# mahyarnajibi/SNIPER

Measured on AMD Instinct MI355X. Metric: train chips/sec (512x512, R101), higher is better.
Workload: dtype f16; 1 GPU; ResNet-101 Faster-RCNN SNIPER 3-scale, batch 20 x 512x512 fp16 per GPU (BASELINE configs[1]); step = GPU anchor labelling + fwd + bwd + grad all-reduce + SGD on HBM-resident chips (epoch chip generation / box assignment and image decode+resize are outside the step); f16 MFMA operands, f32 accumulation / losses / master weights; chips_per_gpu=20, global_batch=20, parallelism=dp1

## Files before the change

### sniper_amd/csrc/nn_ops.hip

```cpp
#include "common.h"
#include "softmax_grad.h"
#include <algorithm>

__global__ __launch_bounds__(256) void pack_stem_kernel(const float *__restrict__ x, half_t *__restrict__ out, int N, int C,
                                                        int H, int W, int Hp, int Wp, int pad_t, int pad_l,
                                                        const float *__restrict__ scale, const float *__restrict__ shift) {
  const long total = (long)N * Hp * Wp;
  for (long i = (long)blockIdx.x * blockDim.x + threadIdx.x; i < total; i += (long)gridDim.x * blockDim.x) {
    const int xp = (int)(i % Wp);
    const long t = i / Wp;
    const int yp = (int)(t % Hp), n = (int)(t / Hp);
    const int sy = yp - pad_t, sx = xp - pad_l;
    half_t v[4] = {0, 0, 0, 0};
    if ((unsigned)sy < (unsigned)H && (unsigned)sx < (unsigned)W) {
      for (int c = 0; c < C && c < 4; ++c) {
        float f = x[(((long)n * C + c) * H + sy) * W + sx];
        if (scale) f = f * scale[c] + shift[c];
        v[c] = (half_t)f;
      }
    }
    *reinterpret_cast<uint2 *>(out + i * 4) = *reinterpret_cast<uint2 *>(v);
  }
}

// ... 1121 lines not shown

__global__ __launch_bounds__(256) void softmax_rows_bwd_kernel(const float *__restrict__ p, const float *__restrict__ label,
                                                               float *__restrict__ g, long outer, int K, int R, SnDiv dK, float ignore,
                                                               int use_ignore, float grad_scale, int normalize_valid,
                                                               const int *__restrict__ valid_count) {
  softmax_bwd_rows(p, label, g, outer, K, R, dK, ignore, use_ignore, softmax_grad_mul(grad_scale, normalize_valid, valid_count));
}

SN_EXPORT int sn_softmax_fwd(const float *x, float *p, long outer, int K, long inner, sn_stream_t stream) {
  SN_REQUIRE(x && p && outer > 0 && K > 0 && inner > 0, "sn_softmax_fwd: bad arguments");
  if (softmax_rows_ok(x, p, K, inner)) {
    const int R = softmax_rows_per_block(K);
    SN_REQUIRE((outer + R - 1) / R < (1l << 31), "sn_softmax_fwd: too many rows");
    hipLaunchKernelGGL(softmax_rows_fwd_kernel, dim3((unsigned)((outer + R - 1) / R)), dim3(256), (size_t)R * (K | 1) * sizeof(float),
                       sn_stream(stream), x, p, outer, K, R, sn_div_make((unsigned)K));
  } else {
    hipLaunchKernelGGL(softmax_fwd_kernel, dim3(ew_blocks(outer * inner)), dim3(256), 0, sn_stream(stream), x, p, outer, K, inner);
  }
  SN_CHECK_LAUNCH();
  return SN_OK;
}

int sn_softmax_count_valid(const float *label, long n, float ignore_label, int use_ignore, int *ws, hipStream_t s) {
  SN_HIP(hipMemsetAsync(ws, 0, sizeof(int), s));
  hipLaunchKernelGGL(count_valid_kernel, dim3(sn_blocks(n, 256)), dim3(256), 0, s, label, n, use_ignore ? ignore_label : -1e30f, ws);
  SN_CHECK_LAUNCH();
  return SN_OK;
}

SN_EXPORT int sn_softmax_output_bwd(const float *p, const float *label, float *grad, long outer, int K, long inner,
                                    float ignore_label, int use_ignore, float grad_scale, int normalize_valid, int *ws,
                                    sn_stream_t stream) {
  SN_REQUIRE(p && label && grad && ws, "sn_softmax_output_bwd: null pointer");
  hipStream_t s = sn_stream(stream);
  if (normalize_valid) {
    const int rc = sn_softmax_count_valid(label, outer * inner, ignore_label, use_ignore, ws, s);
    if (rc != SN_OK) return rc;
  }
  if (softmax_rows_ok(p, grad, K, inner)) {
    const int R = softmax_rows_per_block(K);
    SN_REQUIRE((outer + R - 1) / R < (1l << 31), "sn_softmax_output_bwd: too many rows");
    hipLaunchKernelGGL(softmax_rows_bwd_kernel, dim3((unsigned)((outer + R - 1) / R)), dim3(256), 0, s, p, label, grad, outer, K, R,
                       sn_div_make((unsigned)K), ignore_label, use_ignore, grad_scale, normalize_valid, ws);
  } else {
    hipLaunchKernelGGL(softmax_bwd_kernel, dim3(ew_blocks(outer * inner)), dim3(256), 0, s, p, label, grad, outer, K, inner,
                       ignore_label, use_ignore, grad_scale, normalize_valid, ws);
  }
  SN_CHECK_LAUNCH();
  return SN_OK;
}

__global__ __launch_bounds__(256) void smooth_l1_kernel(const float *__restrict__ pred, const float *__restrict__ target,
                                                        const float *__restrict__ weight, float *__restrict__ loss,
                                                        float *__restrict__ dpred, long n, float sigma, float grad_scale) {
  const float s2 = sigma * sigma, th = 1.f / s2;
  for (long i = (long)blockIdx.x * blockDim.x + threadIdx.x; i < n; i += (long)gridDim.x * blockDim.x) {
    const float d = pred[i] - target[i], w = weight[i];
    const float ad = fabsf(d);
    if (loss) loss[i] = w * (ad < th ? 0.5f * s2 * d * d : ad - 0.5f * th);
    if (dpred) dpred[i] = grad_scale * w * (ad < th ? s2 * d : (d > 0.f ? 1.f : (d < 0.f ? -1.f : 0.f)));
  }
}

SN_EXPORT int sn_smooth_l1_loss(const float *pred, const float *target, const float *weight, float *loss, float *dpred,
                                long n, float sigma, float grad_scale, sn_stream_t stream) {
  SN_REQUIRE(pred && target && weight && n > 0, "sn_smooth_l1_loss: bad arguments");
  hipLaunchKernelGGL(smooth_l1_kernel, dim3(ew_blocks(n)), dim3(256), 0, sn_stream(stream), pred, target, weight, loss, dpred,
                     n, sigma, grad_scale);
  SN_CHECK_LAUNCH();
  return SN_OK;
}

__global__ __launch_bounds__(256) void sgd_kernel(float *__restrict__ w32, const float *__restrict__ grad, float *__restrict__ mom,
                                                  half_t *__restrict__ w16, long n, float lr, float wd, float momentum,
                                                  float rescale) {
  for (long i = (long)blockIdx.x * blockDim.x + threadIdx.x; i < n; i += (long)gridDim.x * blockDim.x) {
    const float w = w32[i];
    const float g = rescale * grad[i] + wd * w;
    const float m = momentum * mom[i] - lr * g;
    mom[i] = m;
    const float nw = w + m;
    w32[i] = nw;
    if (w16) w16[i] = (half_t)nw;
  }
}

SN_EXPORT int sn_sgd_mom_update(float *w32, const float *grad, float *mom, void *w16, long n, float lr, float wd,
                                float momentum, float rescale, sn_stream_t stream) {
  SN_REQUIRE(w32 && grad && mom && n >= 0, "sn_sgd_mom_update: bad arguments");
  if (n == 0) return SN_OK;
  hipLaunchKernelGGL(sgd_kernel, dim3(ew_blocks(n)), dim3(256), 0, sn_stream(stream), w32, grad, mom, (half_t *)w16, n, lr, wd,
                     momentum, rescale);
  SN_CHECK_LAUNCH();
  return SN_OK;
}

__device__ __forceinline__ float sgd_statement(float w, float gr, float m_old, float lr, float wd, float momentum, float rescale,
                                               float &nm) {
  const float g = rescale * gr + wd * w;
  nm = momentum * m_old - lr * g;
  return w + nm;
}

__device__ __forceinline__ float sgd_statement_guarded(float w, float gr, float m_old, float lr, float wd, float momentum, float rescale,
                                                       float coef, float clip, float &nm) {
  float u = rescale * (coef * gr);
  if (clip > 0.f) u = fminf(fmaxf(u, -clip), clip);
  const float g = u + wd * w;
  nm = momentum * m_old - lr * g;
  return w + nm;
}

__global__ __launch_bounds__(256) void sgd_dev_kernel(float *__restrict__ w32, const float *__restrict__ grad,
                                                      float *__restrict__ mom, half_t *__restrict__ w16, long n,
                                                      const float *__restrict__ hyper, float lr_mult, float wd_mult) {
  const float lr = hyper[0] * lr_mult, wd = hyper[1] * wd_mult, momentum = hyper[2], rescale = hyper[3];
  for (long i = (long)blockIdx.x * blockDim.x + threadIdx.x; i < n; i += (long)gridDim.x * blockDim.x) {
    float m;
    const float nw = sgd_statement(w32[i], grad[i], mom[i], lr, wd, momentum, rescale, m);
    mom[i] = m;
    w32[i] = nw;
    if (w16) w16[i] = (half_t)nw;
  }
}

__global__ __launch_bounds__(256) void sgd_dev_vec4_kernel(float4 *__restrict__ w32, const float4 *__restrict__ grad,
                                                           float4 *__restrict__ mom, half_t *__restrict__ w16, long n4,
                                                           const float *__restrict__ hyper, float lr_mult, float wd_mult) {
  const float lr = hyper[0] * lr_mult, wd = hyper[1] * wd_mult, momentum = hyper[2], rescale = hyper[3];
  for (long i = (long)blockIdx.x * blockDim.x + threadIdx.x; i < n4; i += (long)gridDim.x * blockDim.x) {
    const float4 w = w32[i], g4 = grad[i], m4 = mom[i];
    float4 nm, nw;
    nw.x = sgd_statement(w.x, g4.x, m4.x, lr, wd, momentum, rescale, nm.x);
    nw.y = sgd_statement(w.y, g4.y, m4.y, lr, wd, momentum, rescale, nm.y);
    nw.z = sgd_statement(w.z, g4.z, m4.z, lr, wd, momentum, rescale, nm.z);
    nw.w = sgd_statement(w.w, g4.w, m4.w, lr, wd, momentum, rescale, nm.w);
    mom[i] = nm;
    w32[i] = nw;
    if (w16) {
      half4 h;
      h[0] = (half_t)nw.x; h[1] = (half_t)nw.y; h[2] = (half_t)nw.z; h[3] = (half_t)nw.w;
      *reinterpret_cast<half4 *>(w16 + 4 * i) = h;
    }
  }
}

SN_EXPORT int sn_sgd_mom_update_dev(float *w32, const float *grad, float *mom, void *w16, long n, const float *d_hyper,
                                    float lr_mult, float wd_mult, sn_stream_t stream) {
  SN_REQUIRE(w32 && grad && mom && d_hyper && n >= 0, "sn_sgd_mom_update_dev: bad arguments");
  if (n == 0) return SN_OK;
  auto scalar = [&](long from, long count) {
    hipLaunchKernelGGL(sgd_dev_kernel, dim3(ew_blocks(count)), dim3(256), 0, sn_stream(stream), w32 + from, grad + from,
                       mom + from, w16 ? (half_t *)w16 + from : (half_t *)nullptr, count, d_hyper, lr_mult, wd_mult);
  };
  long head = (long)(((16 - ((uintptr_t)w32 & 15)) & 15) / 4);
  if (head > n) head = n;
  const bool same = (((uintptr_t)(w32 + head) | (uintptr_t)(grad + head) | (uintptr_t)(mom + head)) & 15) == 0 &&
                    (w16 == nullptr || ((uintptr_t)((half_t *)w16 + head) & 7) == 0);
  if (!same) {
    scalar(0, n);
    SN_CHECK_LAUNCH();
    return SN_OK;
  }
  if (head > 0) scalar(0, head);
  const long n4 = (n - head) / 4;
  if (n4 > 0)
    hipLaunchKernelGGL(sgd_dev_vec4_kernel, dim3(ew_blocks(n4)), dim3(256), 0, sn_stream(stream), (float4 *)(w32 + head),
                       (const float4 *)(grad + head), (float4 *)(mom + head), w16 ? (half_t *)w16 + head : (half_t *)nullptr, n4,
                       d_hyper, lr_mult, wd_mult);
  const long done = head + 4 * n4;
  if (done < n) scalar(done, n - done);
  SN_CHECK_LAUNCH();
  return SN_OK;
}

__global__ __launch_bounds__(256) void sgd_guard_kernel(float *__restrict__ w32, const float *__restrict__ grad,
                                                        float *__restrict__ mom, half_t *__restrict__ w16, long n,
                                                        const float *__restrict__ hyper, float lr_mult, float wd_mult, float clip,
                                                        const double *__restrict__ state) {
  if (state[2] != 0.0) return;
  const float coef = (float)state[1];
  const float lr = hyper[0] * lr_mult, wd = hyper[1] * wd_mult, momentum = hyper[2], rescale = hyper[3];
  if (coef == 1.f && !(clip > 0.f)) {
    for (long i = (long)blockIdx.x * blockDim.x + threadIdx.x; i < n; i += (long)gridDim.x * blockDim.x) {
      float m;
      const float nw = sgd_statement(w32[i], grad[i], mom[i], lr, wd, momentum, rescale, m);
      mom[i] = m;
      w32[i] = nw;
      if (w16) w16[i] = (half_t)nw;
    }
    return;
  }
  for (long i = (long)blockIdx.x * blockDim.x + threadIdx.x; i < n; i += (long)gridDim.x * blockDim.x) {
    float m;
    const float nw = sgd_statement_guarded(w32[i], grad[i], mom[i], lr, wd, momentum, rescale, coef, clip, m);
    mom[i] = m;
    w32[i] = nw;
    if (w16) w16[i] = (half_t)nw;
  }
}

__global__ __launch_bounds__(256) void sgd_guard_vec4_kernel(float4 *__restrict__ w32, const float4 *__restrict__ grad,
                                                             float4 *__restrict__ mom, half_t *__restrict__ w16, long n4,
                                                             const float *__restrict__ hyper, float lr_mult, float wd_mult,
                                                             float clip, const double *__restrict__ state) {
  if (state[2] != 0.0) return;
  const float coef = (float)state[1];
  const float lr = hyper[0] * lr_mult, wd = hyper[1] * wd_mult, momentum = hyper[2], rescale = hyper[3];
  if (coef == 1.f && !(clip > 0.f)) {
    for (long i = (long)blockIdx.x * blockDim.x + threadIdx.x; i < n4; i += (long)gridDim.x * blockDim.x) {
      const float4 w = w32[i], g4 = grad[i], m4 = mom[i];
      float4 nm, nw;
      nw.x = sgd_statement(w.x, g4.x, m4.x, lr, wd, momentum, rescale, nm.x);
      nw.y = sgd_statement(w.y, g4.y, m4.y, lr, wd, momentum, rescale, nm.y);
      nw.z = sgd_statement(w.z, g4.z, m4.z, lr, wd, momentum, rescale, nm.z);
      nw.w = sgd_statement(w.w, g4.w, m4.w, lr, wd, momentum, rescale, nm.w);
      mom[i] = nm;
      w32[i] = nw;
      if (w16) {
        half4 h;
        h[0] = (half_t)nw.x; h[1] = (half_t)nw.y; h[2] = (half_t)nw.z; h[3] = (half_t)nw.w;
        *reinterpret_cast<half4 *>(w16 + 4 * i) = h;
      }
    }
    return;
  }
  for (long i = (long)blockIdx.x * blockDim.x + threadIdx.x; i < n4; i += (long)gridDim.x * blockDim.x) {
    const float4 w = w32[i], g4 = grad[i], m4 = mom[i];
    float4 nm, nw;
    nw.x = sgd_statement_guarded(w.x, g4.x, m4.x, lr, wd, momentum, rescale, coef, clip, nm.x);
    nw.y = sgd_statement_guarded(w.y, g4.y, m4.y, lr, wd, momentum, rescale, coef, clip, nm.y);
    nw.z = sgd_statement_guarded(w.z, g4.z, m4.z, lr, wd, momentum, rescale, coef, clip, nm.z);
    nw.w = sgd_statement_guarded(w.w, g4.w, m4.w, lr, wd, momentum, rescale, coef, clip, nm.w);
    mom[i] = nm;
    w32[i] = nw;
    if (w16) {
      half4 h;
      h[0] = (half_t)nw.x; h[1] = (half_t)nw.y; h[2] = (half_t)nw.z; h[3] = (half_t)nw.w;
      *reinterpret_cast<half4 *>(w16 + 4 * i) = h;
    }
  }
}

SN_EXPORT int sn_sgd_mom_update_guarded_dev(float *w32, const float *grad, float *mom, void *w16, long n, const float *d_hyper,
                                            float lr_mult, float wd_mult, float clip_gradient, const double *d_state,
                                            sn_stream_t stream) {
  SN_REQUIRE(w32 && grad && mom && d_hyper && d_state && n >= 0, "sn_sgd_mom_update_guarded_dev: bad arguments");
  SN_REQUIRE(clip_gradient == clip_gradient, "sn_sgd_mom_update_guarded_dev: clip_gradient is NaN");
  SN_REQUIRE(((uintptr_t)d_state & 7) == 0, "sn_sgd_mom_update_guarded_dev: d_state must be 8-byte aligned");
  if (n == 0) return SN_OK;
  auto scalar = [&](long from, long count) {
    hipLaunchKernelGGL(sgd_guard_kernel, dim3(ew_blocks(count)), dim3(256), 0, sn_stream(stream), w32 + from, grad + from,
                       mom + from, w16 ? (half_t *)w16 + from : (half_t *)nullptr, count, d_hyper, lr_mult, wd_mult, clip_gradient,
                       d_state);
  };
  long head = (long)(((16 - ((uintptr_t)w32 & 15)) & 15) / 4);
  if (head > n) head = n;
  const bool same = (((uintptr_t)(w32 + head) | (uintptr_t)(grad + head) | (uintptr_t)(mom + head)) & 15) == 0 &&
                    (w16 == nullptr || ((uintptr_t)((half_t *)w16 + head) & 7) == 0);
  if (!same) {
    scalar(0, n);
    SN_CHECK_LAUNCH();
    return SN_OK;
  }
  if (head > 0) scalar(0, head);
  const long n4 = (n - head) / 4;
  if (n4 > 0)
    hipLaunchKernelGGL(sgd_guard_vec4_kernel, dim3(ew_blocks(n4)), dim3(256), 0, sn_stream(stream), (float4 *)(w32 + head),
                       (const float4 *)(grad + head), (float4 *)(mom + head), w16 ? (half_t *)w16 + head : (half_t *)nullptr, n4,
                       d_hyper, lr_mult, wd_mult, clip_gradient, d_state);
  const long done = head + 4 * n4;
  if (done < n) scalar(done, n - done);
  SN_CHECK_LAUNCH();
  return SN_OK;
}

__global__ __launch_bounds__(256) void weight_oti_to_ito_kernel(const float *__restrict__ w, half_t *__restrict__ wt, int O, int T,
                                                                int I, int Opad) {
  const long total = (long)Opad * T * I;
  for (long i = (long)blockIdx.x * blockDim.x + threadIdx.x; i < total; i += (long)gridDim.x * blockDim.x) {
    const int o = (int)(i % Opad);
    const long r = i / Opad;
    const int t = (int)(r % T), ci = (int)(r / T);
    wt[i] = o < O ? (half_t)w[((long)o * T + t) * I + ci] : (half_t)0;
  }
}

SN_EXPORT int sn_weight_transpose(const float *w_oti, void *wt_ito_f16, int O, int T, int I, int O_pad, sn_stream_t stream) {
  SN_REQUIRE(w_oti && wt_ito_f16 && O > 0 && T > 0 && I > 0 && O_pad >= O, "sn_weight_transpose: bad arguments");
  hipLaunchKernelGGL(weight_oti_to_ito_kernel, dim3(ew_blocks((long)O_pad * T * I)), dim3(256), 0, sn_stream(stream), w_oti,
                     (half_t *)wt_ito_f16, O, T, I, O_pad);
  SN_CHECK_LAUNCH();
  return SN_OK;
}

struct WtDesc {
  const float *src;
  half_t *dst;
  int O, T, I, Opad, tile0, tiles_o, tiles_i, pad_;
};
static_assert(sizeof(WtDesc) == 48, "WtDesc layout is part of the C ABI (sn_weight_transpose_batched)");

__global__ __launch_bounds__(256) void weight_transpose_batched_kernel(const WtDesc *__restrict__ desc, int nd) {
  __shared__ float sm[64][65];
  const int tile = blockIdx.x;
  int lo = 0, hi = nd - 1;
  while (lo < hi) {
    const int mid = (lo + hi + 1) >> 1;
    if (desc[mid].tile0 <= tile) lo = mid; else hi = mid - 1;
  }
  const WtDesc d = desc[lo];
  const int local = tile - d.tile0, per_t = d.tiles_o * d.tiles_i;
  const int t = local / per_t, rem = local - t * per_t;
  const int o0 = (rem / d.tiles_i) * 64, i0 = (rem % d.tiles_i) * 64;
  const int c = threadIdx.x & 63, r = threadIdx.x >> 6;
#pragma unroll
  for (int k = 0; k < 16; ++k) {
    const int o = o0 + r + 4 * k, ci = i0 + c;
    sm[r + 4 * k][c] = (o < d.O && ci < d.I) ? d.src[((size_t)o * d.T + t) * d.I + ci] : 0.f;
  }
  __syncthreads();
#pragma unroll
  for (int k = 0; k < 16; ++k) {
    const int ci = i0 + r + 4 * k, o = o0 + c;
    if (ci < d.I && o < d.Opad) d.dst[((size_t)ci * d.T + t) * d.Opad + o] = (half_t)sm[c][r + 4 * k];
  }
}

SN_EXPORT int sn_weight_transpose_batched(const void *desc, int n_desc, int total_tiles, sn_stream_t stream) {
  SN_REQUIRE(desc && n_desc > 0 && total_tiles > 0, "sn_weight_transpose_batched: bad arguments");
  hipLaunchKernelGGL(weight_transpose_batched_kernel, dim3(total_tiles), dim3(256), 0, sn_stream(stream), (const WtDesc *)desc,
                     n_desc);
  SN_CHECK_LAUNCH();
  return SN_OK;
}

__global__ __launch_bounds__(256) void ew_f32_kernel(const float *__restrict__ a, const float *__restrict__ b, float *__restrict__ out,
                                                     long n, int op, float scalar) {
  for (long i = (long)blockIdx.x * blockDim.x + threadIdx.x; i < n; i += (long)gridDim.x * blockDim.x) {
    float v;
    switch (op) {
      case 0: v = a[i] - b[i]; break;
      case 1: v = a[i] + b[i]; break;
      case 2: v = a[i] * b[i]; break;
      case 3: v = a[i] * scalar; break;
      default: v = scalar; break;
    }
    out[i] = v;
  }
}

SN_EXPORT int sn_ew_f32(const float *a, const float *b, float *out, long n, int op, float scalar, sn_stream_t stream) {
  SN_REQUIRE(out && n > 0 && op >= 0 && op <= 4, "sn_ew_f32: bad arguments");
  SN_REQUIRE(op == 4 || a, "sn_ew_f32: null a");
  SN_REQUIRE(op > 2 || b, "sn_ew_f32: null b");
  hipLaunchKernelGGL(ew_f32_kernel, dim3(ew_blocks(n)), dim3(256), 0, sn_stream(stream), a, b, out, n, op, scalar);
  SN_CHECK_LAUNCH();
  return SN_OK;
}

template <typename T>
__global__ __launch_bounds__(256) void bias_grad_kernel(const T *__restrict__ dy, float *__restrict__ db, float *__restrict__ part,
                                                        long rows, int C, int ld, long rows_per_block) {
  const long r0 = (long)blockIdx.y * rows_per_block, r1 = min(rows, r0 + rows_per_block);
  const int c = blockIdx.x * 64 + (threadIdx.x & 63);
  const int rl = threadIdx.x >> 6;
  float s = 0.f;
  if (c < C)
    for (long r = r0 + rl; r < r1; r += 4) s += (float)dy[r * ld + c];
  __shared__ float red[4][64];
  red[rl][threadIdx.x & 63] = s;
  __syncthreads();
  if (rl == 0 && c < C) {
    const float t = (red[0][threadIdx.x] + red[1][threadIdx.x]) + (red[2][threadIdx.x] + red[3][threadIdx.x]);
    if (part) part[(size_t)blockIdx.y * C + c] = t;
    else db[c] += t;
  }
}

__global__ __launch_bounds__(256) void bias_grad_vec8_kernel(const half_t *__restrict__ dy, float *__restrict__ db, float *__restrict__ part,
                                                             long rows, int C, int ld, long rows_per_block) {
  const long r0 = (long)blockIdx.y * rows_per_block, r1 = min(rows, r0 + rows_per_block);
  const int lane = threadIdx.x & 63, rl = threadIdx.x >> 6;
  const int c = (blockIdx.x * 64 + lane) * 8;
  float s[8] = {0.f, 0.f, 0.f, 0.f, 0.f, 0.f, 0.f, 0.f};
  if (c < C) {
    long r = r0 + rl;
    for (; r + 12 < r1; r += 16) {
      half8 v[4];
#pragma unroll
      for (int u = 0; u < 4; ++u) v[u] = *reinterpret_cast<const half8 *>(dy + (r + 4 * u) * ld + c);
#pragma unroll
      for (int u = 0; u < 4; ++u)
#pragma unroll
        for (int j = 0; j < 8; ++j) s[j] += (float)v[u][j];
    }
    for (; r < r1; r += 4) {
      const half8 v = *reinterpret_cast<const half8 *>(dy + r * ld + c);
#pragma unroll
      for (int j = 0; j < 8; ++j) s[j] += (float)v[j];
    }
  }
  __shared__ float red[4][64][9];
#pragma unroll
  for (int j = 0; j < 8; ++j) red[rl][lane][j] = s[j];
  __syncthreads();
  if (rl == 0 && c < C) {
#pragma unroll
    for (int j = 0; j < 8; ++j) {
      if (c + j >= C) break;
      const float t = (red[0][lane][j] + red[1][lane][j]) + (red[2][lane][j] + red[3][lane][j]);
      if (part) part[(size_t)blockIdx.y * C + c + j] = t;
      else db[c + j] += t;
    }
  }
}

static int bias_grad_blocks(long rows, long *rows_per_block) {
  int by = (int)((rows + 255) / 256);
  if (by > 96) by = 96;
  if (by < 1) by = 1;
  *rows_per_block = (rows + by - 1) / by;
  return (int)((rows + *rows_per_block - 1) / *rows_per_block);
}

SN_EXPORT size_t sn_bias_grad_workspace_bytes(long rows, int C) {
  if (rows <= 0 || C <= 0) return 0;
  long rpb;
  int by = bias_grad_blocks(rows, &rpb);
  if (by > 1) by = (int)std::max<long>(by, std::min<long>(128, (rows + 63) / 64));
  return by > 1 ? sn_align(sizeof(float) * (size_t)by * C) : 0;
}

SN_EXPORT int sn_bias_grad(const void *dy, float *db, long rows, int C, int ld, int dtype, void *ws, size_t ws_bytes,
                           sn_stream_t stream) {
  SN_REQUIRE(dy && db && rows > 0 && C > 0, "sn_bias_grad: bad arguments");
  long rpb;
  int by = bias_grad_blocks(rows, &rpb);
  const bool vec8 = dtype == 0 && ld % 8 == 0 && sn_div_up(C, 8) * 8 <= ld && ((uintptr_t)dy % 16) == 0;
  if (vec8 && by > 1 && sn_div_up(C, 512) * by < 256) {
    by = (int)std::min<long>(std::min<long>(128, (rows + 63) / 64), by * 4L);
    if (ws && ws_bytes < sizeof(float) * (size_t)by * C) by = bias_grad_blocks(rows, &rpb);
    rpb = (rows + by - 1) / by;
  }
  float *part = nullptr;
  if (by > 1) {
    if (ws && ws_bytes >= sizeof(float) * (size_t)by * C) part = (float *)ws;
    else { by = 1; rpb = rows; }
  }
  dim3 grid(sn_div_up(C, 64), by);
  hipStream_t s = sn_stream(stream);
  if (vec8)
    hipLaunchKernelGGL(bias_grad_vec8_kernel, dim3(sn_div_up(C, 512), by), dim3(256), 0, s, (const half_t *)dy, db, part, rows, C, ld, rpb);
  else if (dtype == 0)
    hipLaunchKernelGGL((bias_grad_kernel<half_t>), grid, dim3(256), 0, s, (const half_t *)dy, db, part, rows, C, ld, rpb);
  else
    hipLaunchKernelGGL((bias_grad_kernel<float>), grid, dim3(256), 0, s, (const float *)dy, db, part, rows, C, ld, rpb);
  SN_CHECK_LAUNCH();
  return part ? sn_partial_sum(part, by, C, db, s) : SN_OK;
}
```

### sniper_amd/csrc/proposal.hip

```cpp
#include "common.h"

extern "C" int sn_nms_batch(const float *, const int32_t *, int, int, int, float, int, void *, int32_t *, int32_t *, sn_stream_t);
extern "C" size_t sn_nms_workspace_bytes(int, int);

struct PropLayout {
  int total, sort_n, pre, post;
  size_t boxes_all, keys, sorted, nvalid, keep, nkeep, nms, bytes;
};

static int next_pow2(int v) { int p = 1; while (p < v) p <<= 1; return p; }

static PropLayout prop_layout(int B, int A, int Fh, int Fw, int pre, int post) {
  PropLayout L;
  L.total = A * Fh * Fw;
  L.sort_n = next_pow2(L.total);
  L.pre = pre < L.total ? pre : L.total;
  L.post = post < L.pre ? post : L.pre;
  size_t off = 0;
  L.boxes_all = off; off += sn_align((size_t)B * L.total * 4 * sizeof(float));
  L.keys = off; off += sn_align((size_t)B * L.sort_n * sizeof(unsigned long long));
  L.sorted = off; off += sn_align((size_t)B * L.pre * 5 * sizeof(float));
  L.nvalid = off; off += sn_align((size_t)B * sizeof(int32_t));
  L.keep = off; off += sn_align((size_t)B * L.post * sizeof(int32_t));
  L.nkeep = off; off += sn_align((size_t)B * sizeof(int32_t));
  L.nms = off; off += sn_nms_workspace_bytes(B, L.pre);
  L.bytes = off;
  return L;
}

SN_EXPORT size_t sn_proposal_workspace_bytes(int B, int A, int Fh, int Fw, int pre_nms_top_n, int post_nms_top_n) {
  return prop_layout(B, A, Fh, Fw, pre_nms_top_n, post_nms_top_n).bytes;
}

__global__ __launch_bounds__(256) void proposal_decode_kernel(const float *__restrict__ cls_prob, const float *__restrict__ bbox_pred,
                                                              const float *__restrict__ im_info, const float *__restrict__ base,
                                                              int A, int Fh, int Fw, int stride, float min_size, int total, int sort_n,
                                                              float *__restrict__ boxes_all, unsigned long long *__restrict__ keys) {
  const int b = blockIdx.y;
  const int i = blockIdx.x * blockDim.x + threadIdx.x;
  if (i >= sort_n) return;
  unsigned long long *kb = keys + (size_t)b * sort_n;
  if (i >= total) { kb[i] = ~0ull; return; }
  const int cell = i / A, a = i - cell * A;
  const int h = cell / Fw, w = cell - h * Fw;
  const int FF = Fh * Fw;
  const float score0 = cls_prob[((size_t)b * 2 + 1) * A * FF + (size_t)a * FF + cell];
  const float *bp = bbox_pred + ((size_t)b * 4 * A + 4 * a) * FF + cell;
  const float dx = bp[0], dy = bp[FF], dw = bp[2 * FF], dh = bp[3 * FF];
  const float ax1 = base[4 * a] + (float)(w * stride), ay1 = base[4 * a + 1] + (float)(h * stride);
  const float ax2 = base[4 * a + 2] + (float)(w * stride), ay2 = base[4 * a + 3] + (float)(h * stride);
  const float aw = ax2 - ax1 + 1.0f, ah = ay2 - ay1 + 1.0f;
  const float cx = ax1 + 0.5f * (aw - 1.0f), cy = ay1 + 0.5f * (ah - 1.0f);
  const float pcx = dx * aw + cx, pcy = dy * ah + cy;
  const float pw = (float)exp((double)dw) * aw, ph = (float)exp((double)dh) * ah;
  float x1 = pcx - 0.5f * (pw - 1.0f), y1 = pcy - 0.5f * (ph - 1.0f);
  float x2 = pcx + 0.5f * (pw - 1.0f), y2 = pcy + 0.5f * (ph - 1.0f);
  const float im_h = im_info[3 * b], im_w = im_info[3 * b + 1], im_s = im_info[3 * b + 2];
  x1 = fmaxf(fminf(x1, im_w - 1.0f), 0.f); y1 = fmaxf(fminf(y1, im_h - 1.0f), 0.f);
  x2 = fmaxf(fminf(x2, im_w - 1.0f), 0.f); y2 = fmaxf(fminf(y2, im_h - 1.0f), 0.f);
  float score = score0;
  const float ms = min_size * im_s;
  if ((x2 - x1 + 1.0f) < ms || (y2 - y1 + 1.0f) < ms) score = -1.0f;
  float *o = boxes_all + ((size_t)b * total + i) * 4;
  o[0] = x1; o[1] = y1; o[2] = x2; o[3] = y2;
  kb[i] = ((unsigned long long)(~sn_float_key(score)) << 32) | (unsigned)i;
}

__global__ __launch_bounds__(1024) void bitonic_sort_kernel(unsigned long long *__restrict__ keys, int n) {
  unsigned long long *k = keys + (size_t)blockIdx.x * n;
  for (int size = 2; size <= n; size <<= 1) {
    for (int j = size >> 1; j > 0; j >>= 1) {
      for (int t = threadIdx.x; t < (n >> 1); t += blockDim.x) {
        const int lo = 2 * t - (t & (j - 1));
        const int hi = lo + j;
        const bool up = (lo & size) == 0;
        const unsigned long long a = k[lo], c = k[hi];
        if ((a > c) == up) { k[lo] = c; k[hi] = a; }
      }
      __syncthreads();
    }
  }
}

constexpr int kSelThreads = 1024, kSelRegKeys = 32;
template <bool REG>
__global__ __launch_bounds__(kSelThreads) void topk_select_sort_kernel(unsigned long long *__restrict__ keys, int n, int K, int P2) {
  extern __shared__ __attribute__((aligned(16))) unsigned long long sel_buf[];
  __shared__ unsigned hist[256];
  __shared__ unsigned long long s_prefix, s_mask;
  __shared__ int s_need, s_cnt, s_done;
  unsigned long long *k = keys + (size_t)blockIdx.x * n;
  const int tid = threadIdx.x;
  unsigned long long kreg[REG ? kSelRegKeys : 1];
  if constexpr (REG) {
#pragma unroll
    for (int u = 0; u < kSelRegKeys; ++u) {
      const int i = u * kSelThreads + tid;
      kreg[u] = i < n ? k[i] : 0ull;
    }
  }
  const int iters = REG ? (n + kSelThreads - 1) / kSelThreads : 0;
  if (tid == 0) { s_prefix = 0ull; s_mask = 0ull; s_need = K; s_cnt = 0; s_done = 0; }
  __syncthreads();
  for (int shift = 56; shift >= 0; shift -= 8) {
    if (tid < 256) hist[tid] = 0u;
    __syncthreads();
    if (s_done) break;
    const unsigned long long prefix = s_prefix, mask = s_mask;
    auto count = [&](unsigned long long key, bool valid) {
      const bool in = valid && (key & mask) == prefix;
      const unsigned d = (unsigned)(key >> shift) & 255u;
      const unsigned long long act = __ballot(in);
      if (act) {
        const int leader = __ffsll((long long)act) - 1;
        const unsigned d0 = (unsigned)__shfl((int)d, leader, 64);
        const bool same = __ballot(in && d == d0) == act;
        if (same) {
          if ((int)(threadIdx.x & 63) == leader) atomicAdd(&hist[d0], (unsigned)__popcll(act));
        } else if (in) {
          atomicAdd(&hist[d], 1u);
        }
      }
    };
    if constexpr (REG) {
#pragma unroll
      for (int u = 0; u < kSelRegKeys; ++u)
        if (u < iters) count(kreg[u], u * kSelThreads + tid < n);
    }
    for (int base = 0; !REG && base < n; base += kSelThreads * 8) {
      unsigned long long kk[8];
#pragma unroll
      for (int u = 0; u < 8; ++u) {
        const int i = base + u * kSelThreads + tid;
        kk[u] = i < n ? k[i] : 0ull;
      }
#pragma unroll
      for (int u = 0; u < 8; ++u) count(kk[u], base + u * kSelThreads + tid < n);
    }
    __syncthreads();
    if (tid == 0) {
      int need = s_need, d = 0;
      unsigned cum = 0;
      for (; d < 256; ++d) {
        if (cum + hist[d] >= (unsigned)need) break;
        cum += hist[d];
      }
      s_need = need - (int)cum;
      s_prefix = prefix | ((unsigned long long)d << shift);
      s_mask = mask | (0xFFull << shift);
      if (hist[d] == (unsigned)(need - (int)cum)) {
        s_done = 1;
        s_prefix |= (shift ? ((1ull << shift) - 1ull) : 0ull);
        s_mask = ~0ull;
      }
    }
    __syncthreads();
  }
  __syncthreads();
  const unsigned long long kth = s_prefix;
  for (int i = tid; i < P2; i += kSelThreads) sel_buf[i] = ~0ull;
  __syncthreads();
  if constexpr (REG) {
#pragma unroll
    for (int u = 0; u < kSelRegKeys; ++u)
      if (u * kSelThreads + tid < n && kreg[u] <= kth) {
        const int pos = atomicAdd(&s_cnt, 1);
        if (pos < P2) sel_buf[pos] = kreg[u];
      }
  }
  for (int base = 0; !REG && base < n; base += kSelThreads * 8) {
    unsigned long long kk[8];
#pragma unroll
    for (int u = 0; u < 8; ++u) {
      const int i = base + u * kSelThreads + tid;
      kk[u] = i < n ? k[i] : ~0ull;
    }
#pragma unroll
    for (int u = 0; u < 8; ++u)
      if (base + u * kSelThreads + tid < n && kk[u] <= kth) {
        const int pos = atomicAdd(&s_cnt, 1);
        if (pos < P2) sel_buf[pos] = kk[u];
      }
  }
  __syncthreads();
  for (int size = 2; size <= P2; size <<= 1) {
    for (int j = size >> 1; j > 0; j >>= 1) {
      for (int t = tid; t < (P2 >> 1); t += kSelThreads) {
        const int lo = 2 * t - (t & (j - 1));
        const int hi = lo + j;
        const bool up = (lo & size) == 0;
        const unsigned long long a = sel_buf[lo], c = sel_buf[hi];
        if ((a > c) == up) { sel_buf[lo] = c; sel_buf[hi] = a; }
      }
      __syncthreads();
    }
  }
  for (int i = tid; i < K; i += kSelThreads) k[i] = sel_buf[i];
}

__global__ __launch_bounds__(256) void proposal_gather_kernel(const float *__restrict__ boxes_all, const unsigned long long *__restrict__ keys,
                                                              int total, int sort_n, int pre, float *__restrict__ sorted,
                                                              int32_t *__restrict__ nvalid) {
  const int b = blockIdx.y;
  const int r = blockIdx.x * blockDim.x + threadIdx.x;
  if (r >= pre) return;
  const unsigned long long key = keys[(size_t)b * sort_n + r];
  const unsigned idx = (unsigned)(key & 0xffffffffu);
  const unsigned ob = ~(unsigned)(key >> 32);
  const unsigned u = (ob & 0x80000000u) ? (ob & 0x7fffffffu) : ~ob;
  const float *s = boxes_all + ((size_t)b * total + idx) * 4;
  float *o = sorted + ((size_t)b * pre + r) * 5;
  o[0] = s[0]; o[1] = s[1]; o[2] = s[2]; o[3] = s[3]; o[4] = __uint_as_float(u);
  if (r == 0) nvalid[b] = pre;
}

__global__ __launch_bounds__(256) void proposal_output_kernel(const float *__restrict__ sorted, const int32_t *__restrict__ keep,
                                                              const int32_t *__restrict__ nkeep, int pre, int post,
                                                              float *__restrict__ rois, float *__restrict__ scores) {
  const int b = blockIdx.y;
  const int k = blockIdx.x * blockDim.x + threadIdx.x;
  if (k >= post) return;
  const int nk = max(nkeep[b], 1);
  const int src = keep[(size_t)b * post + (k % nk)];
  const float *s = sorted + ((size_t)b * pre + src) * 5;
  float *o = rois + ((size_t)b * post + k) * 5;
  o[0] = (float)b; o[1] = s[0]; o[2] = s[1]; o[3] = s[2]; o[4] = s[3];
  if (scores) scores[(size_t)b * post + k] = s[4];
}

__global__ __launch_bounds__(256) void proposal_target_kernel(const float *__restrict__ rois, const float *__restrict__ gt_boxes,
                                                              const float *__restrict__ valid_ranges, int G, int post,
                                                              float fg_thresh, float4 stds, float *__restrict__ label,
                                                              float *__restrict__ bbox_target, float *__restrict__ bbox_weight,
                                                              float *__restrict__ match) {
  const int b = blockIdx.y;
  const int k = blockIdx.x * blockDim.x + threadIdx.x;
  extern __shared__ __attribute__((aligned(16))) float sgt[];
  const float lo = valid_ranges[2 * b], hi = valid_ranges[2 * b + 1];
  for (int g = threadIdx.x; g < G; g += blockDim.x) {
    const float *p = gt_boxes + ((size_t)b * G + g) * 5;
    const float size = sqrtf((p[2] - p[0] + 1.0f) * (p[3] - p[1] + 1.0f));
    sgt[6 * g + 0] = p[0]; sgt[6 * g + 1] = p[1]; sgt[6 * g + 2] = p[2]; sgt[6 * g + 3] = p[3]; sgt[6 * g + 4] = p[4];
    sgt[6 * g + 5] = (p[4] < 0.f) ? -1.f : ((size >= lo && size <= hi) ? 1.f : 0.f);
  }
  __syncthreads();
  if (k >= post) return;
  const float *r = rois + ((size_t)b * post + k) * 5;
  const float x1 = r[1], y1 = r[2], x2 = r[3], y2 = r[4];
  const float area = (x2 - x1 + 1.0f) * (y2 - y1 + 1.0f);
  float best_v = -1.f, best_i = -1.f;
  int arg = -1;
  for (int g = 0; g < G; ++g) {
    const float flag = sgt[6 * g + 5];
    if (flag < 0.f) continue;
    const float gx1 = sgt[6 * g], gy1 = sgt[6 * g + 1], gx2 = sgt[6 * g + 2], gy2 = sgt[6 * g + 3];
    const float iw = fminf(x2, gx2) - fmaxf(x1, gx1) + 1.0f;
    float ov = 0.f;
    if (iw > 0.f) {
      const float ih = fminf(y2, gy2) - fmaxf(y1, gy1) + 1.0f;
      if (ih > 0.f) ov = iw * ih / (area + (gx2 - gx1 + 1.0f) * (gy2 - gy1 + 1.0f) - iw * ih);
    }
    if (flag > 0.f) { if (ov > best_v) { best_v = ov; arg = g; } }
    else if (ov > best_i) best_i = ov;
  }
  float lab = 0.f, t[4] = {0.f, 0.f, 0.f, 0.f}, wv = 0.f;
  if (arg >= 0 && best_v >= fg_thresh) {
    lab = sgt[6 * arg + 4];
    wv = 1.f;
    const float gx1 = sgt[6 * arg], gy1 = sgt[6 * arg + 1], gx2 = sgt[6 * arg + 2], gy2 = sgt[6 * arg + 3];
    const float ew = x2 - x1 + 1.0f, eh = y2 - y1 + 1.0f;
    const float ecx = x1 + 0.5f * (ew - 1.0f), ecy = y1 + 0.5f * (eh - 1.0f);
    const float gw = gx2 - gx1 + 1.0f, gh = gy2 - gy1 + 1.0f;
    const float gcx = gx1 + 0.5f * (gw - 1.0f), gcy = gy1 + 0.5f * (gh - 1.0f);
    t[0] = (gcx - ecx) / (ew + 1e-7f) / stds.x;
    t[1] = (gcy - ecy) / (eh + 1e-7f) / stds.y;
    t[2] = logf(gw / (ew + 1e-7f)) / stds.z;
    t[3] = logf(gh / (eh + 1e-7f)) / stds.w;
  } else if (best_i >= fg_thresh) {
    lab = -1.f;
  }
  const size_t o = (size_t)b * post + k;
  label[o] = lab;
  if (match) match[o] = wv > 0.f ? (float)arg : -1.f;
#pragma unroll
  for (int c = 0; c < 4; ++c) { bbox_target[4 * o + c] = t[c]; bbox_weight[4 * o + c] = wv; }
}

static int proposal_common(const float *cls_prob, const float *bbox_pred, const float *im_info, const float *base_anchors, int B,
                           int A, int Fh, int Fw, int stride, int pre, int post, float nms_thresh, float min_size, char *ws,
                           const PropLayout &L, hipStream_t s) {
  float *boxes_all = (float *)(ws + L.boxes_all);
  unsigned long long *keys = (unsigned long long *)(ws + L.keys);
  float *sorted = (float *)(ws + L.sorted);
  int32_t *nvalid = (int32_t *)(ws + L.nvalid);
  int32_t *keep = (int32_t *)(ws + L.keep);
  int32_t *nkeep = (int32_t *)(ws + L.nkeep);
  hipLaunchKernelGGL(proposal_decode_kernel, dim3(sn_div_up(L.sort_n, 256), B), dim3(256), 0, s, cls_prob, bbox_pred, im_info,
                     base_anchors, A, Fh, Fw, stride, min_size, L.total, L.sort_n, boxes_all, keys);
  SN_CHECK_LAUNCH();
  const int P2 = next_pow2(L.pre);
  if (P2 <= 16384 && L.pre < L.sort_n && !sn_debug_get(SN_OPT_PROPOSAL_FULL_SORT)) {
    if (L.sort_n <= kSelRegKeys * kSelThreads) {
      SN_HIP(sn_once_per_device_max_lds(reinterpret_cast<const void *>(topk_select_sort_kernel<true>), 16384 * 8));
      hipLaunchKernelGGL(topk_select_sort_kernel<true>, dim3(B), dim3(kSelThreads), (size_t)P2 * 8, s, keys, L.sort_n, L.pre, P2);
    } else {
      SN_HIP(sn_once_per_device_max_lds(reinterpret_cast<const void *>(topk_select_sort_kernel<false>), 16384 * 8));
      hipLaunchKernelGGL(topk_select_sort_kernel<false>, dim3(B), dim3(kSelThreads), (size_t)P2 * 8, s, keys, L.sort_n, L.pre, P2);
    }
  } else {
    hipLaunchKernelGGL(bitonic_sort_kernel, dim3(B), dim3(1024), 0, s, keys, L.sort_n);
  }
  SN_CHECK_LAUNCH();
  hipLaunchKernelGGL(proposal_gather_kernel, dim3(sn_div_up(L.pre, 256), B), dim3(256), 0, s, boxes_all, keys, L.total, L.sort_n,
                     L.pre, sorted, nvalid);
  SN_CHECK_LAUNCH();
  return sn_nms_batch(sorted, nvalid, B, L.pre, 5, nms_thresh, L.post, ws + L.nms, keep, nkeep, (sn_stream_t)s);
}

SN_EXPORT int sn_multi_proposal(const float *cls_prob, const float *bbox_pred, const float *im_info, const float *base_anchors,
                                int B, int A, int Fh, int Fw, int feat_stride, int pre_nms_top_n, int post_nms_top_n, float nms_thresh,
                                float min_size, void *ws, float *rois, float *scores, sn_stream_t stream) {
  SN_REQUIRE(cls_prob && bbox_pred && im_info && base_anchors && ws && rois && B > 0 && A > 0 && Fh > 0 && Fw > 0,
             "sn_multi_proposal: bad arguments");
  const PropLayout L = prop_layout(B, A, Fh, Fw, pre_nms_top_n, post_nms_top_n);
  hipStream_t s = sn_stream(stream);
  if (int rc = proposal_common(cls_prob, bbox_pred, im_info, base_anchors, B, A, Fh, Fw, feat_stride, L.pre, L.post, nms_thresh,
                               min_size, (char *)ws, L, s))
    return rc;
  hipLaunchKernelGGL(proposal_output_kernel, dim3(sn_div_up(L.post, 256), B), dim3(256), 0, s,
                     (const float *)((char *)ws + L.sorted), (const int32_t *)((char *)ws + L.keep),
                     (const int32_t *)((char *)ws + L.nkeep), L.pre, L.post, rois, scores);
  SN_CHECK_LAUNCH();
  return SN_OK;
}

SN_EXPORT int sn_multi_proposal_target(const float *cls_prob, const float *bbox_pred, const float *im_info, const float *gt_boxes,
                                       const float *valid_ranges, const float *base_anchors, int B, int A, int Fh, int Fw,
                                       int feat_stride, int G, int pre_nms_top_n, int post_nms_top_n, float nms_thresh,
                                       float min_size, float fg_thresh, const float *bbox_stds4, void *ws, float *rois,
                                       float *label, float *bbox_target, float *bbox_weight, sn_stream_t stream) {
  SN_REQUIRE(gt_boxes && valid_ranges && label && bbox_target && bbox_weight && bbox_stds4 && G > 0 && G <= 1024,
             "sn_multi_proposal_target: bad arguments");
  if (int rc = sn_multi_proposal(cls_prob, bbox_pred, im_info, base_anchors, B, A, Fh, Fw, feat_stride, pre_nms_top_n, post_nms_top_n,
                                 nms_thresh, min_size, ws, rois, nullptr, stream))
    return rc;
  const PropLayout L = prop_layout(B, A, Fh, Fw, pre_nms_top_n, post_nms_top_n);
  const float4 stds = make_float4(bbox_stds4[0], bbox_stds4[1], bbox_stds4[2], bbox_stds4[3]);
  hipLaunchKernelGGL(proposal_target_kernel, dim3(sn_div_up(L.post, 256), B), dim3(256), (size_t)G * 6 * sizeof(float),
                     sn_stream(stream), rois, gt_boxes, valid_ranges, G, L.post, fg_thresh, stds, label, bbox_target, bbox_weight,
                     (float *)nullptr);
  SN_CHECK_LAUNCH();
  return SN_OK;
}

__global__ __launch_bounds__(256) void mask_rois_select_kernel(const float *__restrict__ rois, const float *__restrict__ label,
                                                               const float *__restrict__ match, int post, int nm,
                                                               float *__restrict__ mask_rois, float *__restrict__ mask_ids) {
  __shared__ int wave_cnt[4];
  __shared__ int taken_s;
  const int b = blockIdx.x, tid = threadIdx.x, lane = tid & 63, wave = tid >> 6;
  const unsigned long long lt = (1ull << lane) - 1ull;
  if (tid == 0) taken_s = 0;
  __syncthreads();
  for (int base = 0; base < post; base += 256) {
    const int k = base + tid;
    const bool fg = k < post && label[(size_t)b * post + k] > 0.f;
    const unsigned long long m = __ballot(fg);
    if (lane == 0) wave_cnt[wave] = __popcll(m);
    __syncthreads();
    int off = taken_s, total = 0;
#pragma unroll
    for (int w = 0; w < 4; ++w) {
      off += w < wave ? wave_cnt[w] : 0;
      total += wave_cnt[w];
    }
    const int slot = off + __popcll(m & lt);
    if (fg && slot < nm) {
      const float *r = rois + ((size_t)b * post + k) * 5;
      float *o = mask_rois + ((size_t)b * nm + slot) * 5;
      o[0] = r[0]; o[1] = r[1]; o[2] = r[2]; o[3] = r[3]; o[4] = r[4];
      mask_ids[(size_t)b * nm + slot] = match[(size_t)b * post + k];
    }
    __syncthreads();
    if (tid == 0) taken_s += total;
    __syncthreads();
    if (taken_s >= nm) break;
  }
  for (int slot = min(taken_s, nm) + tid; slot < nm; slot += 256) {
    float *o = mask_rois + ((size_t)b * nm + slot) * 5;
    o[0] = (float)b; o[1] = 0.f; o[2] = 0.f; o[3] = 0.f; o[4] = 0.f;
    mask_ids[(size_t)b * nm + slot] = -1.f;
  }
}

SN_EXPORT int sn_multi_proposal_target_mask(const float *cls_prob, const float *bbox_pred, const float *im_info, const float *gt_boxes,
                                            const float *valid_ranges, const float *base_anchors, int B, int A, int Fh, int Fw,
                                            int feat_stride, int G, int pre_nms_top_n, int post_nms_top_n, float nms_thresh,
                                            float min_size, float fg_thresh, const float *bbox_stds4, void *ws, float *match_ws,
                                            int num_mask_rois, float *rois, float *label, float *bbox_target, float *bbox_weight,
                                            float *mask_rois, float *mask_ids, sn_stream_t stream) {
  SN_REQUIRE(gt_boxes && valid_ranges && label && bbox_target && bbox_weight && bbox_stds4 && G > 0 && G <= 1024 && match_ws &&
                 mask_rois && mask_ids && num_mask_rois > 0, "sn_multi_proposal_target_mask: bad arguments");
  if (int rc = sn_multi_proposal(cls_prob, bbox_pred, im_info, base_anchors, B, A, Fh, Fw, feat_stride, pre_nms_top_n, post_nms_top_n,
                                 nms_thresh, min_size, ws, rois, nullptr, stream))
    return rc;
  const PropLayout L = prop_layout(B, A, Fh, Fw, pre_nms_top_n, post_nms_top_n);
  const float4 stds = make_float4(bbox_stds4[0], bbox_stds4[1], bbox_stds4[2], bbox_stds4[3]);
  hipLaunchKernelGGL(proposal_target_kernel, dim3(sn_div_up(L.post, 256), B), dim3(256), (size_t)G * 6 * sizeof(float),
                     sn_stream(stream), rois, gt_boxes, valid_ranges, G, L.post, fg_thresh, stds, label, bbox_target, bbox_weight,
                     match_ws);
  SN_CHECK_LAUNCH();
  hipLaunchKernelGGL(mask_rois_select_kernel, dim3(B), dim3(256), 0, sn_stream(stream), rois, label, match_ws, L.post, num_mask_rois,
                     mask_rois, mask_ids);
  SN_CHECK_LAUNCH();
  return SN_OK;
}
```

Before: 1003 chips/s.

## Vectorize weight transpose via swizzled f16 LDS and register-resident bitonic top-k sort

The batched weight transpose now reads source rows as float4, converts to f16 before staging in an XOR-swizzled half-precision LDS tile, and writes output as 16-byte vectors, with scalar fallbacks for unaligned shapes. Separately, the proposal top-k sort replaces the all-shared-memory bitonic network with a register-blocked bitonic sort that uses in-register compare-exchange, wave shuffles for mid strides, and LDS only for large strides. Both aim to cut memory transactions and barriers in small per-step kernels, at the cost of more complex indexing and higher register pressure.

```diff
diff --git a/sniper_amd/csrc/nn_ops.hip b/sniper_amd/csrc/nn_ops.hip
--- a/sniper_amd/csrc/nn_ops.hip
+++ b/sniper_amd/csrc/nn_ops.hip
@@ -1447,7 +1447,7 @@
 static_assert(sizeof(WtDesc) == 48, "WtDesc layout is part of the C ABI (sn_weight_transpose_batched)");
 
 __global__ __launch_bounds__(256) void weight_transpose_batched_kernel(const WtDesc *__restrict__ desc, int nd) {
-  __shared__ float sm[64][65];
+  __shared__ __attribute__((aligned(16))) half_t sm[64 * 64];
   const int tile = blockIdx.x;
   int lo = 0, hi = nd - 1;
   while (lo < hi) {
@@ -1458,17 +1458,47 @@
   const int local = tile - d.tile0, per_t = d.tiles_o * d.tiles_i;
   const int t = local / per_t, rem = local - t * per_t;
   const int o0 = (rem / d.tiles_i) * 64, i0 = (rem % d.tiles_i) * 64;
-  const int c = threadIdx.x & 63, r = threadIdx.x >> 6;
-#pragma unroll
-  for (int k = 0; k < 16; ++k) {
-    const int o = o0 + r + 4 * k, ci = i0 + c;
-    sm[r + 4 * k][c] = (o < d.O && ci < d.I) ? d.src[((size_t)o * d.T + t) * d.I + ci] : 0.f;
+  const bool vec_src = (d.I & 3) == 0 && ((uintptr_t)d.src & 15) == 0;
+  const bool vec_dst = (d.Opad & 7) == 0 && ((uintptr_t)d.dst & 15) == 0;
+  const int c4 = threadIdx.x & 15, og = threadIdx.x >> 4;
+  float v[4][4];
+#pragma unroll
+  for (int r = 0; r < 4; ++r) {
+    const int o = o0 + 4 * og + r, ci = i0 + 4 * c4;
+    const float *row = d.src + ((size_t)o * d.T + t) * d.I;
+    if (vec_src) {
+      const float4 q = (o < d.O && ci < d.I) ? *reinterpret_cast<const float4 *>(row + ci) : make_float4(0.f, 0.f, 0.f, 0.f);
+      v[r][0] = q.x; v[r][1] = q.y; v[r][2] = q.z; v[r][3] = q.w;
+    } else {
+#pragma unroll
+      for (int k = 0; k < 4; ++k) v[r][k] = (o < d.O && ci + k < d.I) ? row[ci + k] : 0.f;
+    }
+  }
+#pragma unroll
+  for (int k = 0; k < 4; ++k) {
+    union { half_t h[4]; uint2 u; } p;
+#pragma unroll
+    for (int r = 0; r < 4; ++r) p.h[r] = (half_t)v[r][k];
+    *reinterpret_cast<uint2 *>(sm + (4 * c4 + k) * 64 + ((og ^ c4) << 2)) = p.u;
   }
   __syncthreads();
 #pragma unroll
-  for (int k = 0; k < 16; ++k) {
-    const int ci = i0 + r + 4 * k, o = o0 + c;
-    if (ci < d.I && o < d.Opad) d.dst[((size_t)ci * d.T + t) * d.Opad + o] = (half_t)sm[c][r + 4 * k];
+  for (int p = 0; p < 2; ++p) {
+    const int idx = threadIdx.x + 256 * p, i = idx >> 3, c = idx & 7, s = (i >> 2) & 15;
+    uint4 q = *reinterpret_cast<const uint4 *>(sm + i * 64 + ((c ^ (s >> 1)) << 3));
+    if (s & 1) q = make_uint4(q.z, q.w, q.x, q.y);
+    const int ci = i0 + i, o = o0 + 8 * c;
+    if (ci >= d.I || o >= d.Opad) continue;
+    half_t *out = d.dst + ((size_t)ci * d.T + t) * d.Opad + o;
+    if (vec_dst) {
+      *reinterpret_cast<uint4 *>(out) = q;
+    } else {
+      union { uint4 u; half_t h[8]; } w;
+      w.u = q;
+#pragma unroll
+      for (int k = 0; k < 8; ++k)
+        if (o + k < d.Opad) out[k] = w.h[k];
+    }
   }
 }
 
diff --git a/sniper_amd/csrc/proposal.hip b/sniper_amd/csrc/proposal.hip
--- a/sniper_amd/csrc/proposal.hip
+++ b/sniper_amd/csrc/proposal.hip
@@ -83,6 +83,69 @@
 }
 
 constexpr int kSelThreads = 1024, kSelRegKeys = 32;
+
+template <int E>
+__device__ __forceinline__ void sorted_prefix_store(unsigned long long *buf, unsigned long long *__restrict__ out, int K, int P2) {
+  const int tid = threadIdx.x, base = tid * E;
+  unsigned long long v[E];
+  auto cex = [](unsigned long long &a, unsigned long long &c, bool up) {
+    const bool sw = (a > c) == up;
+    const unsigned long long x = sw ? c : a;
+    c = sw ? a : c;
+    a = x;
+  };
+#pragma unroll
+  for (int e = 0; e < E; ++e) v[e] = buf[e * kSelThreads + tid];
+#pragma unroll
+  for (int size = 2; size <= E; size <<= 1)
+#pragma unroll
+    for (int j = size >> 1; j > 0; j >>= 1)
+#pragma unroll
+      for (int e = 0; e < E; ++e)
+        if ((e & j) == 0) cex(v[e], v[e | j], ((base + e) & size) == 0);
+  for (int size = 2 * E; size <= P2; size <<= 1) {
+    const bool up = (base & size) == 0;
+    int j = size >> 1;
+    if (j >= 64 * E) {
+#pragma unroll
+      for (int e = 0; e < E; ++e) buf[e * kSelThreads + tid] = v[e];
+      __syncthreads();
+      for (; j >= 64 * E; j >>= 1) {
+        const int jt = j / E;
+        for (int q = tid; q < (P2 >> 1); q += kSelThreads) {
+          const int e = q / (kSelThreads / 2), r = q % (kSelThreads / 2);
+          const int tlo = 2 * r - (r & (jt - 1));
+          unsigned long long *p = buf + e * kSelThreads + tlo;
+          const unsigned long long a = p[0], c = p[jt];
+          if ((a > c) == (((tlo * E) & size) == 0)) { p[0] = c; p[jt] = a; }
+        }
+        __syncthreads();
+      }
+#pragma unroll
+      for (int e = 0; e < E; ++e) v[e] = buf[e * kSelThreads + tid];
+    }
+    for (; j >= E; j >>= 1) {
+      const int m = j / E;
+      const bool keep_min = ((tid & m) == 0) == up;
+#pragma unroll
+      for (int e = 0; e < E; ++e) {
+        const unsigned long long o = __shfl_xor(v[e], m, 64);
+        v[e] = ((v[e] < o) == keep_min) ? v[e] : o;
+      }
+    }
+#pragma unroll
+    for (int jj = E >> 1; jj > 0; jj >>= 1)
+#pragma unroll
+      for (int e = 0; e < E; ++e)
+        if ((e & jj) == 0) cex(v[e], v[e | jj], up);
+  }
+  __syncthreads();
+#pragma unroll
+  for (int e = 0; e < E; ++e) buf[base + e] = v[e];
+  __syncthreads();
+  for (int i = tid; i < K; i += kSelThreads) out[i] = buf[i];
+}
+
 template <bool REG>
 __global__ __launch_bounds__(kSelThreads) void topk_select_sort_kernel(unsigned long long *__restrict__ keys, int n, int K, int P2) {
   extern __shared__ __attribute__((aligned(16))) unsigned long long sel_buf[];
@@ -183,6 +246,14 @@
       }
   }
   __syncthreads();
+  switch (P2 / kSelThreads) {
+    case 16: sorted_prefix_store<16>(sel_buf, k, K, P2); return;
+    case 8: sorted_prefix_store<8>(sel_buf, k, K, P2); return;
+    case 4: sorted_prefix_store<4>(sel_buf, k, K, P2); return;
+    case 2: sorted_prefix_store<2>(sel_buf, k, K, P2); return;
+    case 1: sorted_prefix_store<1>(sel_buf, k, K, P2); return;
+    default: break;
+  }
   for (int size = 2; size <= P2; size <<= 1) {
     for (int j = size >> 1; j > 0; j >>= 1) {
       for (int t = tid; t < (P2 >> 1); t += kSelThreads) {
```

Measured after the change: 1006 chips/s (median of 4 runs). About the same (+0.2%).
